# nagadomi/nunif

Hardware: NVIDIA H100
Metric: waifu2x_input_megapixels_per_sec (higher is better)
Workload: dtype f16

## Files before the change

### nunif_b200/csrc/gemm_wgmma.cuh

```cuda
#pragma once
#include "common.cuh"
#include <cuda.h>

namespace nb200 {

enum : int { ACT_NONE = 0, ACT_LRELU01 = 1, ACT_GELU = 2, ACT_RELU = 3 };
enum : int { OUT_NHWC = 0, OUT_PIXSHUF2 = 1, OUT_SPLIT = 2 };

struct GemmParams {
    int B, Ho, Wo, TH, TW, tiles_x, tiles_y;
    int N;
    int taps, cpt;
    int8_t tap_dx[16], tap_dy[16], tap_dyi[16];
    int n_tiles;
    const float* bias;
    int act;
    int out_mode, cout;
    int has_res, res_cy, res_cx;
    int res_before_act;
};

struct GemmMaps {
    CUtensorMap a, b;
    CUtensorMap o[4];
    CUtensorMap r[4];
};

__device__ __forceinline__ uint32_t smem_u32(const void* p) { return (uint32_t)__cvta_generic_to_shared(p); }

__device__ __forceinline__ void mbar_init(uint64_t* bar, uint32_t count) {
    asm volatile("mbarrier.init.shared::cta.b64 [%0], %1;" ::"r"(smem_u32(bar)), "r"(count));
}
__device__ __forceinline__ void mbar_expect_tx(uint64_t* bar, uint32_t bytes) {
    asm volatile("mbarrier.arrive.expect_tx.shared::cta.b64 _, [%0], %1;" ::"r"(smem_u32(bar)), "r"(bytes) : "memory");
}
__device__ __forceinline__ void mbar_arrive(uint64_t* bar) {
    asm volatile("mbarrier.arrive.shared::cta.b64 _, [%0];" ::"r"(smem_u32(bar)) : "memory");
}
static __device__ __noinline__ void mbar_timeout() {
    printf("nb200: mbarrier wait timed out (block %d,%d thread %d)\n", blockIdx.x, blockIdx.y, threadIdx.x);
    __trap();
}
__device__ __forceinline__ void mbar_wait(uint64_t* bar, uint32_t parity) {
    const uint32_t addr = smem_u32(bar);
    uint32_t done = 0;
#pragma unroll 1
    for (uint32_t it = 0; it < (1u << 18); ++it) {
        asm volatile(
            "{\n\t.reg .pred p;\n\t"
            "mbarrier.try_wait.parity.shared::cta.b64 p, [%1], %2, %3;\n\t"
            "selp.u32 %0, 1, 0, p;\n\t}"
            : "=r"(done) : "r"(addr), "r"(parity), "r"(20000u) : "memory");
        if (done) return;
    }
    mbar_timeout();
}
__device__ __forceinline__ void fence_barrier_init() {
    asm volatile("fence.mbarrier_init.release.cluster;" ::: "memory");
    asm volatile("fence.proxy.async.shared::cta;" ::: "memory");
}
__device__ __forceinline__ void tma_load_5d(const CUtensorMap* map, uint64_t* bar, void* dst, int c0, int c1, int c2, int c3, int c4) {
    asm volatile(
        "cp.async.bulk.tensor.5d.shared::cluster.global.tile.mbarrier::complete_tx::bytes [%0], [%1, {%3, %4, %5, %6, %7}], [%2];"
        ::"r"(smem_u32(dst)), "l"(map), "r"(smem_u32(bar)), "r"(c0), "r"(c1), "r"(c2), "r"(c3), "r"(c4) : "memory");
}
__device__ __forceinline__ void tma_load_2d(const CUtensorMap* map, uint64_t* bar, void* dst, int c0, int c1) {
    asm volatile(
        "cp.async.bulk.tensor.2d.shared::cluster.global.tile.mbarrier::complete_tx::bytes [%0], [%1, {%3, %4}], [%2];"
        ::"r"(smem_u32(dst)), "l"(map), "r"(smem_u32(bar)), "r"(c0), "r"(c1) : "memory");
}
__device__ __forceinline__ void tma_load_4d(const CUtensorMap* map, uint64_t* bar, void* dst, int c0, int c1, int c2, int c3) {
    asm volatile(
        "cp.async.bulk.tensor.4d.shared::cluster.global.tile.mbarrier::complete_tx::bytes [%0], [%1, {%3, %4, %5, %6}], [%2];"
        ::"r"(smem_u32(dst)), "l"(map), "r"(smem_u32(bar)), "r"(c0), "r"(c1), "r"(c2), "r"(c3) : "memory");
}
__device__ __forceinline__ void tma_store_4d(const CUtensorMap* map, const void* src, int c0, int c1, int c2, int c3) {
    asm volatile("cp.async.bulk.tensor.4d.global.shared::cta.tile.bulk_group [%0, {%2, %3, %4, %5}], [%1];"
                 ::"l"(map), "r"(smem_u32(src)), "r"(c0), "r"(c1), "r"(c2), "r"(c3) : "memory");
}
__device__ __forceinline__ void tma_store_2d(const CUtensorMap* map, const void* src, int c0, int c1) {
    asm volatile("cp.async.bulk.tensor.2d.global.shared::cta.tile.bulk_group [%0, {%2, %3}], [%1];"
                 ::"l"(map), "r"(smem_u32(src)), "r"(c0), "r"(c1) : "memory");
}
__device__ __forceinline__ void tma_store_commit() { asm volatile("cp.async.bulk.commit_group;" ::: "memory"); }
__device__ __forceinline__ void tma_store_wait_read() { asm volatile("cp.async.bulk.wait_group.read 0;" ::: "memory"); }
__device__ __forceinline__ void fence_async_smem() { asm volatile("fence.proxy.async.shared::cta;" ::: "memory"); }
__device__ __forceinline__ void consumer_bar_sync() { asm volatile("bar.sync 1, 256;" ::: "memory"); }
__device__ __forceinline__ void tma_prefetch_desc(const CUtensorMap* map) {
    asm volatile("prefetch.tensormap [%0];" ::"l"(map) : "memory");
}
__device__ __forceinline__ bool elect_one() {
    uint32_t pred;
    asm volatile(
        "{\n\t.reg .pred p;\n\t"
        "elect.sync _|p, 0xffffffff;\n\t"
        "selp.u32 %0, 1, 0, p;\n\t}"
        : "=r"(pred));
    return pred != 0;
}
__device__ __forceinline__ void wgmma_fence() { asm volatile("wgmma.fence.sync.aligned;" ::: "memory"); }
__device__ __forceinline__ void wgmma_commit() { asm volatile("wgmma.commit_group.sync.aligned;" ::: "memory"); }
template <int N>
__device__ __forceinline__ void wgmma_wait() { asm volatile("wgmma.wait_group.sync.aligned %0;" ::"n"(N) : "memory"); }
template <int K>
__device__ __forceinline__ void wgmma_fence_operands(float (&d)[K]) {
#pragma unroll
    for (int j = 0; j < K; ++j) asm volatile("" : "+f"(d[j])::"memory");
}

template <int SWIZZLE_BYTES>
__device__ __forceinline__ uint64_t make_kmajor_desc(uint32_t saddr) {
    constexpr uint64_t layout = SWIZZLE_BYTES == 128 ? 1 : (SWIZZLE_BYTES == 64 ? 2 : 3);
    constexpr uint64_t sbo = (8 * SWIZZLE_BYTES) >> 4;
    return (uint64_t)((saddr & 0x3FFFF) >> 4) | (1ull << 16) | (sbo << 32) | (layout << 62);
}

template <int N>
__device__ void wgmma_f16(float (&d)[N / 2], uint64_t a, uint64_t b, uint32_t acc);
template <> __device__ __forceinline__ void wgmma_f16<16>(float (&d)[8], uint64_t a, uint64_t b, uint32_t acc) {
    asm volatile("{\n\t.reg .pred p;\n\tsetp.ne.b32 p, %10, 0;\n\t"
                 "wgmma.mma_async.sync.aligned.m64n16k16.f32.f16.f16 {%0, %1, %2, %3, %4, %5, %6, %7}, %8, %9, p, 1, 1, 0, 0;\n\t}"
                 : "+f"(d[0]), "+f"(d[1]), "+f"(d[2]), "+f"(d[3]), "+f"(d[4]), "+f"(d[5]), "+f"(d[6]), "+f"(d[7])
                 : "l"(a), "l"(b), "r"(acc));
}
template <> __device__ __forceinline__ void wgmma_f16<32>(float (&d)[16], uint64_t a, uint64_t b, uint32_t acc) {
    asm volatile("{\n\t.reg .pred p;\n\tsetp.ne.b32 p, %18, 0;\n\t"
                 "wgmma.mma_async.sync.aligned.m64n32k16.f32.f16.f16 {%0, %1, %2, %3, %4, %5, %6, %7, %8, %9, %10, %11, %12, %13, %14, %15}, %16, %17, p, 1, 1, 0, 0;\n\t}"
                 : "+f"(d[0]), "+f"(d[1]), "+f"(d[2]), "+f"(d[3]), "+f"(d[4]), "+f"(d[5]), "+f"(d[6]), "+f"(d[7]), "+f"(d[8]), "+f"(d[9]), "+f"(d[10]), "+f"(d[11]), "+f"(d[12]), "+f"(d[13]), "+f"(d[14]), "+f"(d[15])
                 : "l"(a), "l"(b), "r"(acc));
}
template <> __device__ __forceinline__ void wgmma_f16<48>(float (&d)[24], uint64_t a, uint64_t b, uint32_t acc) {
    asm volatile("{\n\t.reg .pred p;\n\tsetp.ne.b32 p, %26, 0;\n\t"
                 "wgmma.mma_async.sync.aligned.m64n48k16.f32.f16.f16 {%0, %1, %2, %3, %4, %5, %6, %7, %8, %9, %10, %11, %12, %13, %14, %15, %16, %17, %18, %19, %20, %21, %22, %23}, %24, %25, p, 1, 1, 0, 0;\n\t}"
                 : "+f"(d[0]), "+f"(d[1]), "+f"(d[2]), "+f"(d[3]), "+f"(d[4]), "+f"(d[5]), "+f"(d[6]), "+f"(d[7]), "+f"(d[8]), "+f"(d[9]), "+f"(d[10]), "+f"(d[11]), "+f"(d[12]), "+f"(d[13]), "+f"(d[14]), "+f"(d[15]), "+f"(d[16]), "+f"(d[17]), "+f"(d[18]), "+f"(d[19]), "+f"(d[20]), "+f"(d[21]), "+f"(d[22]), "+f"(d[23])
                 : "l"(a), "l"(b), "r"(acc));
}
template <> __device__ __forceinline__ void wgmma_f16<64>(float (&d)[32], uint64_t a, uint64_t b, uint32_t acc) {
    asm volatile("{\n\t.reg .pred p;\n\tsetp.ne.b32 p, %34, 0;\n\t"
// ... 222 lines not shown
```

### nunif_b200/csrc/swin_attention_mma.cu

```cuda
#include "common.cuh"
#include "gemm_wgmma.cuh"
#include "swin_kernels.h"
#include "tmap.h"
#include <map>
#include <mutex>

namespace nb200 {

extern int g_tune[16];

namespace {
constexpr int WS = 6, WTOK = 36, WPAD = 48, HEADS = 6;

__device__ __forceinline__ void mma16816(float (&c)[4], const uint32_t (&a)[4], uint32_t b0, uint32_t b1) {
    asm volatile(
        "mma.sync.aligned.m16n8k16.row.col.f32.f16.f16.f32 {%0,%1,%2,%3}, {%4,%5,%6,%7}, {%8,%9}, {%0,%1,%2,%3};"
        : "+f"(c[0]), "+f"(c[1]), "+f"(c[2]), "+f"(c[3])
        : "r"(a[0]), "r"(a[1]), "r"(a[2]), "r"(a[3]), "r"(b0), "r"(b1));
}
__device__ __forceinline__ void ldmatrix_x2_trans(uint32_t& r0, uint32_t& r1, const void* smem_row) {
    const uint32_t addr = (uint32_t)__cvta_generic_to_shared(smem_row);
    asm volatile("ldmatrix.sync.aligned.m8n8.x2.trans.shared.b16 {%0,%1}, [%2];" : "=r"(r0), "=r"(r1) : "r"(addr));
}
__device__ __forceinline__ uint32_t pack_half2(float a, float b) {
// ... 194 lines not shown
    AttnCtx<D> cx;
    cx.sq = sq; cx.sreg = sreg; cx.bf = bf; cx.hc = hc; cx.g = g; cx.t4 = t4; cx.scale = scale; cx.boundary = boundary;
#pragma unroll
    for (int nt = 0; nt < NKT; ++nt) cx.kbase[nt] = sk + min(nt * 8 + g, WTOK - 1) * LD + hc + 2 * t4;
    cx.vbase[0] = sv + (lane & 15) * LD + hc;
    cx.vbase[1] = sv + (16 + (lane & 15)) * LD + hc;
    cx.vbase[2] = sv + min(32 + (lane & 7), WTOK - 1) * LD + hc;
#pragma unroll 1
    for (int mt = 0; mt < 2; ++mt) attn_mtile<D, LD, false>(cx, mt);
    attn_mtile<D, LD, true>(cx, 2);
    __syncthreads();
    for (int t = rg; t < WTOK; t += RG)
        *reinterpret_cast<uint4*>(out + (size_t)stok[t] * C + vv * 8) = *reinterpret_cast<const uint4*>(sq + t * LD + vv * 8);
}

__global__ void build_bias_frag_kernel(const float* __restrict__ table, float4* __restrict__ frag) {
    const int i = blockIdx.x * blockDim.x + threadIdx.x;
    if (i >= HEADS * 3 * 6 * 32) return;
    const int lane = i & 31, nt = (i >> 5) % 6, mt = (i / (32 * 6)) % 3, head = i / (32 * 6 * 3);
    const int g = lane >> 2, t4 = lane & 3;
    float v[4];
#pragma unroll
    for (int r = 0; r < 4; ++r) {
        const int row = mt * 16 + g + 8 * (r >> 1), col = nt * 8 + 2 * t4 + (r & 1);
        if (col >= WTOK) v[r] = -1e30f;
        else if (row >= WTOK) v[r] = 0.f;
        else {
            const int qy = row / WS, qx = row % WS, ky = col / WS, kx = col % WS;
            v[r] = 1.4426950408889634f * table[((qy - ky + WS - 1) * (2 * WS - 1) + (qx - kx + WS - 1)) * HEADS + head];
        }
    }
    frag[i] = make_float4(v[0], v[1], v[2], v[3]);
}

int build_bias_frag(cudaStream_t st, const float* table, float* frag) {
    build_bias_frag_kernel<<<(HEADS * 3 * 6 * 32 + 255) / 256, 256, 0, st>>>(table, reinterpret_cast<float4*>(frag));
    NB_LAUNCHED();
    return 0;
}

template <int D>
static size_t attn_smem_bytes() {
    constexpr int C = D * HEADS, LD = C + 8;
    return (size_t)3 * WTOK * LD * 2 + (WTOK + WPAD) * 4 + 16;
}

static int set_attn_attrs(const void* func, size_t smem, int carveout) {
    static std::mutex mu;
    static std::map<std::pair<int, const void*>, int> done;
    int dev = 0;
    NB_CUDA(cudaGetDevice(&dev));
    std::lock_guard<std::mutex> lk(mu);
    int& have = done[{dev, func}];
    if (have != carveout) {
        NB_CUDA(cudaFuncSetAttribute(func, cudaFuncAttributeMaxDynamicSharedMemorySize, (int)smem));
        NB_CUDA(cudaFuncSetAttribute(func, cudaFuncAttributePreferredSharedMemoryCarveout, carveout));
        have = carveout;
    }
    return 0;
}

int window_attention(cudaStream_t st, const __half* qkv, const float* bias_frag_f, __half* out, int B, int H, int W, int C,
                     int shift, size_t plane) {
    const float4* bias_table = reinterpret_cast<const float4*>(bias_frag_f);
    NB_CHECK(H % WS == 0 && W % WS == 0, "feature map must be a multiple of the 6x6 window");
    NB_CHECK(C == 96 || C == 192, "window attention supports C=96 (d=16) and C=192 (d=32)");
    if (WS >= H) shift = 0;
    dim3 grid((H / WS) * (W / WS), B);
    ProfScope ps(st, PC_ATTN, (double)B * H * W * C * 4 * 2, (double)B * H * W * C * 3 * 2, (double)B * H * W * C * 2);
    if (C == 96) {
        const int want = g_tune[6] > 0 ? g_tune[6] : 72;
        if (set_attn_attrs((const void*)window_attention_mma_kernel<16>, attn_smem_bytes<16>(), want)) return 1;
        window_attention_mma_kernel<16><<<grid, 192, attn_smem_bytes<16>(), st>>>(qkv, bias_table, out, H, W, shift, plane);
    } else {
        const int want = g_tune[6] > 0 ? g_tune[6] : 86;
        if (set_attn_attrs((const void*)window_attention_mma_kernel<32>, attn_smem_bytes<32>(), want)) return 1;
        window_attention_mma_kernel<32><<<grid, 192, attn_smem_bytes<32>(), st>>>(qkv, bias_table, out, H, W, shift, plane);
    }
    NB_LAUNCHED();
    return 0;
}


constexpr int FA_ROWS = 128, FA_WIN = 3, FA_THREADS = GEMM_CONSUMER_THREADS + 32, FA_SLOT = 96 * 64, FA_STAGES = 4;
constexpr int FA_LD = 32 + 8;
constexpr int FA_CHUNK_BYTES = FA_WIN * 3 * WTOK * FA_LD * 2;

template <int C>
struct FaCfg {
    static constexpr int X_BYTES = FA_ROWS * C * 2;
    static constexpr int SMEM = X_BYTES + FA_STAGES * FA_SLOT + FA_CHUNK_BYTES + FA_WIN * (WTOK + WPAD) * 4 + 2 * FA_STAGES * 8 + 1024;
};

template <int C>
__global__ void __launch_bounds__(FA_THREADS, 2) swin_attn_fused_kernel(const __grid_constant__ CUtensorMap wmap,
                                                                        const __half* __restrict__ x, const float* __restrict__ bqkv,
                                                                        const float4* __restrict__ bias_frag, __half* __restrict__ out,
                                                                        int H, int W, int shift, int nwin) {
    using Cfg = FaCfg<C>;
    constexpr int D = C / HEADS, KB = C / 32, NCH = C / 32, HPC = 32 / D;
    extern __shared__ uint8_t smem_dyn[];
    uint8_t* smem = reinterpret_cast<uint8_t*>((reinterpret_cast<uintptr_t>(smem_dyn) + 1023) & ~(uintptr_t)1023);
    uint8_t* sx = smem;
    uint8_t* ring = smem + Cfg::X_BYTES;
    __half* sqkv = reinterpret_cast<__half*>(ring + FA_STAGES * FA_SLOT);
    int* stok = reinterpret_cast<int*>(reinterpret_cast<uint8_t*>(sqkv) + FA_CHUNK_BYTES);
    int* sreg = stok + FA_WIN * WTOK;
    uint64_t* full = reinterpret_cast<uint64_t*>(sreg + FA_WIN * WPAD);
    uint64_t* empty = full + FA_STAGES;
    const int tid = threadIdx.x, warp = tid >> 5;
    const int nww = W / WS, nwy = H / WS;
    if (tid < FA_WIN * WPAD) {
        const int w = tid / WPAD, t = tid % WPAD, gw = blockIdx.x * FA_WIN + w;
        int reg = -1;
        if (t < WTOK) {
            int tok = -1;
            if (gw < nwin) {
                const int b = gw / (nww * nwy), r = gw % (nww * nwy), wy = r / nww, wx = r % nww;
                const int ry = wy * WS + t / WS, rx = wx * WS + t % WS;
                const int y = (ry + shift) % H, xx = (rx + shift) % W;
                tok = (b * H + y) * W + xx;
                int hr = 0, wr = 0;
                if (shift > 0) {
                    hr = ry < H - WS ? 0 : (ry < H - shift ? 1 : 2);
                    wr = rx < W - WS ? 0 : (rx < W - shift ? 1 : 2);
                }
                reg = hr * 3 + wr;
            }
            stok[w * WTOK + t] = tok;
        }
        sreg[w * WPAD + t] = reg;
    }
    if (tid == GEMM_CONSUMER_THREADS) {
        tma_prefetch_desc(&wmap);
        for (int s = 0; s < FA_STAGES; ++s) {
            mbar_init(&full[s], 1);
            mbar_init(&empty[s], 2);
        }
        fence_barrier_init();
    }
    __syncthreads();
    if (tid == 0) NB_PDL_TRIGGER();

    if (warp == GEMM_CONSUMER_THREADS / 32) {
        if (elect_one()) {
            for (int i = 0; i < NCH * KB; ++i) {
                const int s = i % FA_STAGES, c = i / KB;
                mbar_wait(&empty[s], ((i / FA_STAGES) & 1) ^ 1);
                mbar_expect_tx(&full[s], FA_SLOT);
#pragma unroll
                for (int m = 0; m < 3; ++m)
                    tma_load_2d(&wmap, &full[s], ring + s * FA_SLOT + m * 32 * 64, (i % KB) * 32, m * C + 32 * c);
            }
        }
        return;
    }

    for (int i = tid; i < FA_ROWS * (C / 8); i += GEMM_CONSUMER_THREADS) {
        const int r = i / (C / 8), u = i % (C / 8);
        uint8_t* dst = sx + (u >> 2) * (FA_ROWS * 64) + stage_off<32>(r, u & 3);
        const int tok = r < FA_WIN * WTOK ? stok[r] : -1;
        if (tok >= 0) cp_async16(dst, x + (size_t)tok * C + u * 8);
        else *reinterpret_cast<uint4*>(dst) = make_uint4(0u, 0u, 0u, 0u);
    }
    asm volatile("cp.async.commit_group;" ::: "memory");
    asm volatile("cp.async.wait_group 0;" ::: "memory");
    fence_async_smem();
    consumer_bar_sync();

    const int wg = tid >> 7, t = tid & 127;
    const int row0 = wg * 64 + (t >> 5) * 16 + ((t & 31) >> 2);
    const int cq = 2 * (t & 3);
    const uint32_t a_base = smem_u32(sx) + wg * 64 * 64;
    const int lane = tid & 31, g = lane >> 2, t4 = lane & 3;
    const float scale = ((D == 16) ? 0.25f : 0.17677669529663687f) * 1.4426950408889634f;
#pragma unroll 1
    for (int c = 0; c < NCH; ++c) {
        float acc[48];
#pragma unroll
        for (int j = 0; j < 48; ++j) acc[j] = 0.f;
#pragma unroll 1
        for (int kb = 0; kb < KB; ++kb) {
            const int it = c * KB + kb, s = it % FA_STAGES;
            mbar_wait(&full[s], (it / FA_STAGES) & 1);
            const uint32_t a = a_base + kb * (FA_ROWS * 64), bb = smem_u32(ring + s * FA_SLOT);
            wgmma_fence();
            wgmma_f16<96>(acc, make_kmajor_desc<64>(a), make_kmajor_desc<64>(bb), 1u);
            wgmma_f16<96>(acc, make_kmajor_desc<64>(a + 32), make_kmajor_desc<64>(bb + 32), 1u);
            wgmma_commit();
            wgmma_wait<1>();
            if (kb > 0 && t == 0) mbar_arrive(&empty[(it - 1) % FA_STAGES]);
        }
        wgmma_wait<0>();
        if (t == 0) mbar_arrive(&empty[(c * KB + KB - 1) % FA_STAGES]);
        wgmma_fence_operands(acc);
        consumer_bar_sync();
#pragma unroll
        for (int j = 0; j < 12; ++j) {
            const int m = j >> 2, col = 8 * (j & 3) + cq;
            const float2 bq = __ldg(reinterpret_cast<const float2*>(bqkv + m * C + 32 * c + col));
#pragma unroll
            for (int i = 0; i < 2; ++i) {
                const int r = row0 + 8 * i;
                if (r < FA_WIN * WTOK) {
                    const int w = r / WTOK, tk = r - w * WTOK;
                    *reinterpret_cast<__half2*>(sqkv + ((w * 3 + m) * WTOK + tk) * FA_LD + col) =
                        __floats2half2_rn(acc[4 * j + 2 * i] + bq.x, acc[4 * j + 2 * i + 1] + bq.y);
                }
            }
        }
        consumer_bar_sync();

#pragma unroll 1
        for (int item = warp; item < 3 * FA_WIN * HPC; item += GEMM_CONSUMER_THREADS / 32) {
            const int mt = item / (FA_WIN * HPC), pr = item - mt * (FA_WIN * HPC), w = pr / HPC, hh = pr - w * HPC;
            const int gw = blockIdx.x * FA_WIN + w;
            if (gw >= nwin) continue;
            const int r = gw % (nww * nwy), wy = r / nww, wx = r % nww, head = c * HPC + hh;
            __half* sq = sqkv + w * 3 * WTOK * FA_LD;
            __half* sk = sq + WTOK * FA_LD;
            __half* sv = sk + WTOK * FA_LD;
            AttnCtx<D> cx;
            cx.sq = sq; cx.sreg = sreg + w * WPAD; cx.bf = bias_frag + (size_t)head * (3 * 6 * 32) + lane;
            cx.hc = hh * D; cx.g = g; cx.t4 = t4; cx.scale = scale;
            cx.boundary = shift > 0 && (wy == nwy - 1 || wx == nww - 1);
#pragma unroll
            for (int nt = 0; nt < NKT; ++nt) cx.kbase[nt] = sk + min(nt * 8 + g, WTOK - 1) * FA_LD + cx.hc + 2 * t4;
            cx.vbase[0] = sv + (lane & 15) * FA_LD + cx.hc;
            cx.vbase[1] = sv + (16 + (lane & 15)) * FA_LD + cx.hc;
            cx.vbase[2] = sv + min(32 + (lane & 7), WTOK - 1) * FA_LD + cx.hc;
            if (mt < 2) attn_mtile<D, FA_LD, false>(cx, mt);
            else attn_mtile<D, FA_LD, true>(cx, 2);
            __syncwarp();
            const int nrow = mt < 2 ? 16 : WTOK - 32;
            for (int e = lane; e < nrow * (D / 8); e += 32) {
                const int tk = 16 * mt + e / (D / 8), u = e % (D / 8);
                *reinterpret_cast<uint4*>(out + (size_t)stok[w * WTOK + tk] * C + head * D + u * 8) =
                    *reinterpret_cast<const uint4*>(sq + tk * FA_LD + cx.hc + u * 8);
            }
        }
    }
}

int swin_attn_fused(cudaStream_t st, const __half* x, const __half* wqkv, const float* bqkv, const float* bias_frag_f, __half* att,
                    int B, int H, int W, int C, int shift) {
    NB_CHECK(x && wqkv && bqkv && bias_frag_f && att, "null pointer");
    NB_CHECK(H % WS == 0 && W % WS == 0, "feature map must be a multiple of the 6x6 window");
    NB_CHECK(C == 96 || C == 192, "fused window attention supports C=96 (d=16) and C=192 (d=32)");
    if (WS >= H) shift = 0;
    const long long nwin = (long long)B * (H / WS) * (W / WS);
    NB_CHECK(nwin > 0 && nwin < (1LL << 31), "window count out of range");
    CUtensorMap wmap;
    const cuuint64_t dims[2] = {(cuuint64_t)C, (cuuint64_t)(3 * C)};
    const cuuint64_t strides[1] = {(cuuint64_t)C * 2};
    const cuuint32_t box[2] = {32, 32};
    if (encode(&wmap, wqkv, 2, dims, strides, box, 64)) return 1;
    const double T = (double)B * H * W;
    ProfScope ps(st, PC_FUSED_ATTN, T * 3.0 * C * C * 2 + T * C * 36 * 4, T * C * 2, T * C * 2);
    const unsigned grid = (unsigned)((nwin + FA_WIN - 1) / FA_WIN);
    const float4* bf = reinterpret_cast<const float4*>(bias_frag_f);
    if (C == 96) {
        if (ensure_dyn_smem((const void*)swin_attn_fused_kernel<96>, FaCfg<96>::SMEM)) return 1;
        swin_attn_fused_kernel<96><<<grid, FA_THREADS, FaCfg<96>::SMEM, st>>>(wmap, x, bqkv, bf, att, H, W, shift, (int)nwin);
    } else {
        if (ensure_dyn_smem((const void*)swin_attn_fused_kernel<192>, FaCfg<192>::SMEM)) return 1;
        swin_attn_fused_kernel<192><<<grid, FA_THREADS, FaCfg<192>::SMEM, st>>>(wmap, x, bqkv, bf, att, H, W, shift, (int)nwin);
    }
    NB_LAUNCHED();
    return 0;
}

}
```

### nunif_b200/csrc/swin_block.cu

```cuda
#include "gemm_wgmma.cuh"
#include "swin_kernels.h"
#include "tmap.h"

namespace nb200 {

constexpr int FM_ROWS = 128, FM_STAGES = 5, FM_THREADS = GEMM_CONSUMER_THREADS + 128;
constexpr int FM_PRODUCER_REGS = 40, FM_CONSUMER_REGS = 232;

template <int C>
struct FmCfg {
    static constexpr int KB = C / 32;
    static constexpr int TILE = FM_ROWS * C * 2;
    static constexpr int STAGE = 128 * C;
    static constexpr int SMEM = 2 * TILE + FM_STAGES * STAGE + (2 * FM_STAGES + KB + 1) * 8 + 1024;
};

struct FmMaps {
    CUtensorMap x, att, wp, w1, w2;
};

template <int K>
__device__ __forceinline__ float (&half96(float (&acc)[K], int h))[48] { return *reinterpret_cast<float(*)[48]>(&acc[48 * h]); }

__device__ __forceinline__ void fm_wait(uint64_t* bar, uint32_t parity) {
    const uint32_t addr = smem_u32(bar);
    uint32_t done = 0;
#pragma unroll 1
    for (uint32_t it = 0; it < (1u << 18) && !done; ++it)
        asm volatile(
            "{\n\t.reg .pred p;\n\t"
            "mbarrier.try_wait.parity.shared::cta.b64 p, [%1], %2, %3;\n\t"
            "selp.u32 %0, 1, 0, p;\n\t}"
            : "=r"(done) : "r"(addr), "r"(parity), "r"(20000u) : "memory");
    if (!done) __trap();
}

__device__ __forceinline__ void wgmma_wait_n(int n) {
    if (n == 0) wgmma_wait<0>();
    else wgmma_wait<1>();
}

template <int C, bool PROJ>
__global__ void __launch_bounds__(FM_THREADS, 1) swin_mlp_fused_kernel(const __grid_constant__ FmMaps maps, const float* __restrict__ bp,
                                                                     const float* __restrict__ b1, const float* __restrict__ b2) {
    using Cfg = FmCfg<C>;
    constexpr int KB = Cfg::KB, NP = (KB + 1) / 2, NH = 2 * C / 64, NHALF = C / 96;
    extern __shared__ uint8_t smem_dyn[];
    uint8_t* smem = reinterpret_cast<uint8_t*>((reinterpret_cast<uintptr_t>(smem_dyn) + 1023) & ~(uintptr_t)1023);
    uint8_t* sx = smem;
    uint8_t* satt = smem + Cfg::TILE;
    uint8_t* ring = smem + 2 * Cfg::TILE;
    uint64_t* full = reinterpret_cast<uint64_t*>(ring + FM_STAGES * Cfg::STAGE);
    uint64_t* empty = full + FM_STAGES;
    uint64_t* abar = empty + FM_STAGES;
    uint64_t* xbar = abar + KB;
    const int tid = threadIdx.x, warp = tid >> 5;
    const int row_base = blockIdx.x * FM_ROWS;
    if (tid == GEMM_CONSUMER_THREADS) {
        tma_prefetch_desc(&maps.x);
        tma_prefetch_desc(&maps.w1);
        tma_prefetch_desc(&maps.w2);
        if (PROJ) {
            tma_prefetch_desc(&maps.att);
            tma_prefetch_desc(&maps.wp);
        }
        for (int s = 0; s < FM_STAGES; ++s) {
            mbar_init(&full[s], 1);
            mbar_init(&empty[s], 2);
        }
        for (int kb = 0; kb < KB; ++kb) mbar_init(&abar[kb], 1);
        mbar_init(xbar, 1);
        fence_barrier_init();
    }
    __syncthreads();

    if (warp >= GEMM_CONSUMER_THREADS / 32) {
        asm volatile("setmaxnreg.dec.sync.aligned.u32 %0;" ::"n"(FM_PRODUCER_REGS));
        if (warp == GEMM_CONSUMER_THREADS / 32 && elect_one()) {
            bool acts = false;
            auto load_acts = [&]() {
                asm volatile("griddepcontrol.wait;" ::: "memory");
                if (PROJ)
                    for (int kb = 0; kb < KB; ++kb) {
                        mbar_expect_tx(&abar[kb], FM_ROWS * 64);
                        tma_load_2d(&maps.att, &abar[kb], satt + kb * (FM_ROWS * 64), kb * 32, row_base);
                    }
                mbar_expect_tx(xbar, Cfg::TILE);
                for (int kb = 0; kb < KB; ++kb) tma_load_2d(&maps.x, xbar, sx + kb * (FM_ROWS * 64), kb * 32, row_base);
                acts = true;
            };
            int it = 0;
            auto push = [&](const CUtensorMap* m, int k0, int n0, int rows, int nbox) {
                if (it == FM_STAGES) load_acts();
                const int s = it % FM_STAGES;
                fm_wait(&empty[s], ((it / FM_STAGES) & 1) ^ 1);
                mbar_expect_tx(&full[s], nbox * rows * 64);
                for (int b = 0; b < nbox; ++b) tma_load_2d(m, &full[s], ring + s * Cfg::STAGE + b * rows * 64, k0 + 32 * b, n0);
                ++it;
            };
            if (PROJ)
                for (int j = 0; j < NP; ++j) push(&maps.wp, 64 * j, 0, C, min(2, KB - 2 * j));
            push(&maps.w1, 0, 0, 64, KB);
            for (int hc = 0; hc < NH; ++hc) {
                if (hc + 1 < NH) push(&maps.w1, 0, (hc + 1) * 64, 64, KB);
                push(&maps.w2, hc * 64, 0, C, 2);
            }
            if (!acts) load_acts();
        }
        return;
    }

    asm volatile("setmaxnreg.inc.sync.aligned.u32 %0;" ::"n"(FM_CONSUMER_REGS));
    const int wg = tid >> 7, t = tid & 127;
    const int row0 = wg * 64 + (t >> 5) * 16 + ((t & 31) >> 2);
    const int cq = 2 * (t & 3);
    const uint32_t x_base = smem_u32(sx) + wg * 64 * 64, att_base = smem_u32(satt) + wg * 64 * 64;
    int it = 0, pending = 0;
    auto take = [&]() -> uint32_t {
        const int s = it % FM_STAGES;
        fm_wait(&full[s], (it / FM_STAGES) & 1);
        return smem_u32(ring + s * Cfg::STAGE);
    };
    auto commit = [&]() {
        wgmma_commit();
        ++it;
        ++pending;
    };
    auto retire = [&](int n) {
        wgmma_wait_n(n);
#pragma unroll
        for (int k = 0; k < FM_STAGES; ++k)
            if (k < pending - n && t == 0) mbar_arrive(&empty[(it - pending + k) % FM_STAGES]);
        pending = min(pending, n);
    };

    if (PROJ) {
        float acc[C / 2];
#pragma unroll
        for (int j = 0; j < C / 2; ++j) acc[j] = 0.f;
        wgmma_fence_operands(acc);
#pragma unroll
        for (int j = 0; j < NP; ++j) {
            const uint32_t bb = take();
#pragma unroll
            for (int kb = 2 * j; kb < 2 * j + 2 && kb < KB; ++kb) fm_wait(&abar[kb], 0);
            wgmma_fence();
#pragma unroll
            for (int kb = 2 * j; kb < 2 * j + 2 && kb < KB; ++kb) {
                const uint32_t a = att_base + kb * (FM_ROWS * 64), b = bb + (kb - 2 * j) * (C * 64);
#pragma unroll
                for (int s = 0; s < 2; ++s)
#pragma unroll
                    for (int h = 0; h < NHALF; ++h)
                        wgmma_f16<96>(half96(acc, h), make_kmajor_desc<64>(a + 32 * s), make_kmajor_desc<64>(b + h * 96 * 64 + 32 * s), 1u);
            }
            commit();
            retire(1);
        }
        retire(0);
        wgmma_fence_operands(acc);
        fm_wait(xbar, 0);
#pragma unroll
        for (int j = 0; j < C / 8; ++j) {
            const int col = 8 * j + cq;
            const float2 bq = __ldg(reinterpret_cast<const float2*>(bp + col));
#pragma unroll
            for (int i = 0; i < 2; ++i) {
                __half2* p = reinterpret_cast<__half2*>(sx + sw64_off<FM_ROWS>(row0 + 8 * i, col));
                const float2 xv = __half22float2(*p);
                *p = __floats2half2_rn(xv.x + (acc[4 * j + 2 * i] + bq.x), xv.y + (acc[4 * j + 2 * i + 1] + bq.y));
            }
        }
        fence_async_smem();
        asm volatile("bar.sync %0, 128;" ::"r"(2 + wg) : "memory");
    } else {
        fm_wait(xbar, 0);
    }

    float oacc[C / 2];
#pragma unroll
    for (int j = 0; j < C / 2; ++j) oacc[j] = 0.f;
    wgmma_fence_operands(oacc);
    float hacc[2][32];
    uint32_t af[4][4];
    auto fc1 = [&](float (&h)[32]) {
#pragma unroll
        for (int j = 0; j < 32; ++j) h[j] = 0.f;
        wgmma_fence_operands(h);
        const uint32_t bb = take();
        wgmma_fence();
#pragma unroll
        for (int kb = 0; kb < KB; ++kb) {
            const uint32_t a = x_base + kb * (FM_ROWS * 64), b = bb + kb * (64 * 64);
            wgmma_f16<64>(h, make_kmajor_desc<64>(a), make_kmajor_desc<64>(b), 1u);
            wgmma_f16<64>(h, make_kmajor_desc<64>(a + 32), make_kmajor_desc<64>(b + 32), 1u);
        }
        commit();
    };
    fc1(hacc[0]);
#pragma unroll
    for (int hc = 0; hc < NH; ++hc) {
        const int buf = hc & 1;
        if (hc + 1 < NH) fc1(hacc[buf ^ 1]);
        retire(hc + 1 < NH ? 1 : 0);
        wgmma_fence_operands(hacc[buf]);
#pragma unroll
        for (int kk = 0; kk < 4; ++kk)
#pragma unroll
            for (int q = 0; q < 4; ++q) {
                const int j = 2 * kk + (q >> 1), i = q & 1;
                const float2 bq = __ldg(reinterpret_cast<const float2*>(b1 + 64 * hc + 8 * j + cq));
                const __half2 h = __floats2half2_rn(gelu_erf(hacc[buf][4 * j + 2 * i] + bq.x), gelu_erf(hacc[buf][4 * j + 2 * i + 1] + bq.y));
                af[kk][q] = *reinterpret_cast<const uint32_t*>(&h);
            }
        const uint32_t bb = take();
        wgmma_fence();
#pragma unroll
        for (int kb = 0; kb < 2; ++kb)
#pragma unroll
            for (int s = 0; s < 2; ++s)
#pragma unroll
                for (int h = 0; h < NHALF; ++h)
                    wgmma_f16_rs96(half96(oacc, h), af[2 * kb + s], make_kmajor_desc<64>(bb + kb * (C * 64) + h * 96 * 64 + 32 * s), 1u);
        commit();
    }
    retire(0);
    wgmma_fence_operands(oacc);
#pragma unroll
    for (int j = 0; j < C / 8; ++j) {
        const int col = 8 * j + cq;
        const float2 bq = __ldg(reinterpret_cast<const float2*>(b2 + col));
#pragma unroll
        for (int i = 0; i < 2; ++i) {
            __half2* p = reinterpret_cast<__half2*>(sx + sw64_off<FM_ROWS>(row0 + 8 * i, col));
            const float2 xv = __half22float2(*p);
            *p = __floats2half2_rn(xv.x + (oacc[4 * j + 2 * i] + bq.x), xv.y + (oacc[4 * j + 2 * i + 1] + bq.y));
        }
    }
    fence_async_smem();
    consumer_bar_sync();
    if (tid == 0) {
        for (int kb = 0; kb < KB; ++kb) tma_store_2d(&maps.x, sx + kb * (FM_ROWS * 64), kb * 32, row_base);
        tma_store_commit();
        tma_store_wait_read();
    }
}

static int map2d(CUtensorMap* m, const void* base, int cols, long long rows, int box_rows) {
    const cuuint64_t dims[2] = {(cuuint64_t)cols, (cuuint64_t)rows};
    const cuuint64_t strides[1] = {(cuuint64_t)cols * 2};
    const cuuint32_t box[2] = {32, (cuuint32_t)box_rows};
    return encode(m, base, 2, dims, strides, box, 64);
}

template <int C, bool PROJ>
static int launch_mlp(cudaStream_t st, unsigned grid, const FmMaps& maps, const float* bp, const float* b1, const float* b2) {
    if (ensure_dyn_smem((const void*)swin_mlp_fused_kernel<C, PROJ>, FmCfg<C>::SMEM)) return 1;
    cudaLaunchConfig_t cfg = {};
    cfg.gridDim = dim3(grid); cfg.blockDim = dim3(FM_THREADS); cfg.dynamicSmemBytes = FmCfg<C>::SMEM;
// ... 49 lines not shown
```

### profiles/ab_swin_attn.py

```python
#!/usr/bin/env python
import argparse
import ctypes
import json
import os
import statistics
import subprocess
import sys
import tempfile

ROOT = os.path.dirname(os.path.dirname(os.path.abspath(__file__)))
sys.path.insert(0, ROOT)

SHAPES = [(240, 96), (120, 192), (60, 192), (240, 192)]
BATCH = 16
REPS = 7
WINDOW_MS = 60.0
FA_THREADS = 288
KERNEL = "_ZN5nb20022swin_attn_fused_kernelILi{C}EEEv14CUtensorMap_stPK6__halfPKfPK6float4PS2_iiii"


def load(path):
    from nunif_b200 import _lib
    lib = ctypes.CDLL(os.path.abspath(path))
    for name in ("nb200_last_error", "nb200_check_device", "nb200_swin_attn_fused_f16"):
        res, args = _lib.SIGNATURES[name]
        getattr(lib, name).restype, getattr(lib, name).argtypes = res, args
    return lib


def check(lib, rc):
    if rc != 0:
        raise RuntimeError(lib.nb200_last_error().decode("utf-8", "replace"))


def call(lib, t, shift):
    import torch
    x, wqkv, bqkv, table, att = t
    B, H, W, C = x.shape
    p = lambda v: ctypes.c_void_p(v.data_ptr())
    check(lib, lib.nb200_swin_attn_fused_f16(p(x), p(wqkv), p(bqkv), p(table), p(att), B, H, W, C, shift,
                                             ctypes.c_void_p(torch.cuda.current_stream().cuda_stream)))


def inputs(H, C, shift, dev):
    import torch
    g = torch.Generator(device="cpu").manual_seed(H * 1000 + C + shift)
    x = torch.randn(BATCH, H, H, C, generator=g).half().to(dev)
    wqkv = (torch.randn(3 * C, C, generator=g) / C ** 0.5).half().to(dev)
    bqkv = (0.1 * torch.randn(3 * C, generator=g)).to(dev)
    table = (0.5 * torch.randn(121, 6, generator=g)).to(dev)
    return x, wqkv, bqkv, table


def window_ms(lib, t, shift, n):
    import torch
    e0, e1 = torch.cuda.Event(enable_timing=True), torch.cuda.Event(enable_timing=True)
    e0.record()
    for _ in range(n):
        call(lib, t, shift)
    e1.record()
    e1.synchronize()
    return e0.elapsed_time(e1) / n


def launch_smem(libs, dev):
    import torch
    from torch.profiler import ProfilerActivity, profile
    out = {}
    with tempfile.TemporaryDirectory() as d:
        for tag, lib in libs.items():
            for C in (96, 192):
                x, wqkv, bqkv, table = inputs(12, C, 0, dev)
                t = (x, wqkv, bqkv, table, torch.empty_like(x))
                with profile(activities=[ProfilerActivity.CUDA]) as prof:
                    call(lib, t, 0)
                    torch.cuda.synchronize()
                path = os.path.join(d, f"{tag}{C}.json")
                prof.export_chrome_trace(path)
                ev = [e for e in json.load(open(path))["traceEvents"]
                      if e.get("cat") == "kernel" and "swin_attn_fused_kernel" in e.get("name", "")]
                a = ev[0]["args"]
                out[(tag, C)] = {"smem": int(a["shared memory"]), "regs_trace": int(a["registers per thread"])}
    return out


def occupancy(so_path, C, smem):
    name = KERNEL.format(C=C)
    cuobjdump = os.path.join(os.environ.get("CUDA_HOME", "/usr/local/cuda"), "bin", "cuobjdump")
    with tempfile.TemporaryDirectory() as d:
        subprocess.run([cuobjdump, "-xelf", "all", os.path.abspath(so_path)], cwd=d, check=True, capture_output=True)
        image = next(b for b in (open(os.path.join(d, f), "rb").read() for f in sorted(os.listdir(d))) if name.encode() in b)
    cu = ctypes.CDLL("libcuda.so.1")

    def ck(rc):
        if rc != 0:
            raise RuntimeError(f"CUDA driver error {rc}")
    mod, fn = ctypes.c_void_p(), ctypes.c_void_p()
    ck(cu.cuModuleLoadData(ctypes.byref(mod), ctypes.c_char_p(image)))
    try:
        ck(cu.cuModuleGetFunction(ctypes.byref(fn), mod, name.encode()))
        ck(cu.cuFuncSetAttribute(fn, 8, ctypes.c_int(smem)))
        regs, n = ctypes.c_int(), ctypes.c_int()
        ck(cu.cuFuncGetAttribute(ctypes.byref(regs), 4, fn))
        ck(cu.cuOccupancyMaxActiveBlocksPerMultiprocessor(ctypes.byref(n), fn, FA_THREADS, ctypes.c_size_t(smem)))
    finally:
        cu.cuModuleUnload(mod)
    return regs.value, n.value


def device_info(index):
    q = subprocess.run(["nvidia-smi", "-i", str(index), "--query-gpu=name,power.limit,clocks.max.sm", "--format=csv,noheader"],
                       capture_output=True, text=True)
    return q.stdout.strip()


def main():
    ap = argparse.ArgumentParser(description=__doc__, formatter_class=argparse.RawDescriptionHelpFormatter)
    ap.add_argument("--base", required=True, help="the build to compare against (libnunif_b200.so)")
    ap.add_argument("--new", default=os.path.join(ROOT, "nunif_b200", "libnunif_b200.so"), help="default: this tree's build")
    ap.add_argument("--out", default=None, help="also write the JSON result here")
    args = ap.parse_args()
    import torch
    from bench import ClockSampler
    dev = torch.device("cuda:0")
    torch.cuda.init()
    torch.zeros(1, device=dev)
    paths = {"base": args.base, "new": args.new}
    libs = {k: load(v) for k, v in paths.items()}
    for lib in libs.values():
        check(lib, lib.nb200_check_device(0))
    info = {"device": torch.cuda.get_device_name(dev), "nvidia_smi": device_info(0), "paths": paths}
    print(f"# {info['device']} | name, power limit, max SM clock: {info['nvidia_smi']}")

    kern = []
    try:
        for (tag, C), s in sorted(launch_smem(libs, dev).items()):
            regs, ctas = occupancy(paths[tag], C, s["smem"])
            kern.append({"build": tag, "C": C, "regs": regs, "dyn_smem": s["smem"], "ctas_per_sm": ctas})
            print(f"# {tag:4s} swin_attn_fused_kernel<{C}>: {regs} registers, {s['smem']} B shared memory/CTA, {ctas} CTA(s)/SM")
    except Exception as e:
        kern.append({"error": f"{type(e).__name__}: {e}"})
        print(f"# occupancy query failed: {type(e).__name__}: {e}")

    rows = []
    with torch.inference_mode(), ClockSampler(0) as clocks:
        for H, C in SHAPES:
            for shift in (0, 3):
                x, wqkv, bqkv, table = inputs(H, C, shift, dev)
                t = {k: (x, wqkv, bqkv, table, torch.full_like(x, 7.0)) for k in libs}
                for k, lib in libs.items():
                    for _ in range(3):
                        call(lib, t[k], shift)
                torch.cuda.synchronize()
                equal = torch.equal(t["base"][4], t["new"][4])
                diff = float((t["base"][4].float() - t["new"][4].float()).abs().max())
                est = max(window_ms(libs["base"], t["base"], shift, 2), window_ms(libs["new"], t["new"], shift, 2))
                n = max(3, int(WINDOW_MS / max(est, 1e-3)))
                ms = {k: [] for k in libs}
                for r in range(REPS):
                    for k in (("base", "new") if r % 2 == 0 else ("new", "base")):
                        ms[k].append(window_ms(libs[k], t[k], shift, n))
                row = {"B": BATCH, "H": H, "W": H, "C": C, "shift": shift, "calls_per_window": n, "equal": equal, "max_abs_diff": diff}
                for k in libs:
                    row[k] = {"median_ms": statistics.median(ms[k]), "min_ms": min(ms[k]), "max_ms": max(ms[k])}
                row["new_over_base"] = row["new"]["median_ms"] / row["base"]["median_ms"]
                rows.append(row)
                b, nw = row["base"], row["new"]
                print(f"{BATCH}x{H}x{H}x{C} shift {shift}: base {b['median_ms']:.4f} ms [{b['min_ms']:.4f}, {b['max_ms']:.4f}]  "
                      f"new {nw['median_ms']:.4f} ms [{nw['min_ms']:.4f}, {nw['max_ms']:.4f}]  new/base {row['new_over_base']:.3f}  "
                      f"outputs {'identical' if equal else f'DIFFER (max |d| {diff:g})'}", flush=True)
                del t, x
    result = {"info": info, "clocks": clocks.summary(), "kernels": kern, "shapes": rows,
              "all_equal": all(r["equal"] for r in rows)}
    print(json.dumps(result))
    if args.out:
        os.makedirs(os.path.dirname(os.path.abspath(args.out)), exist_ok=True)
        with open(args.out, "w") as fh:
            json.dump(result, fh, indent=1)
    return 0 if result["all_equal"] else 1


if __name__ == "__main__":
    sys.exit(main())
```

Before: 54.01.

## Deepen fused attention TMA ring, add PDL launch, unroll k-loop, interleave warp items

Raises the weight ring in the fused Swin attention kernel from 4 to 6 stages and fully unrolls the k-block loop. Launches the kernel with programmatic stream serialization and places griddepcontrol.wait before the consumers read activations, so the prologue can overlap the previous kernel. Assigns attention work items to warps in a serpentine order to balance load, and moves the trapping mbarrier wait into the shared header. The extra stages increase shared memory per CTA, which could lower the number of CTAs resident per SM.

```diff
diff --git a/nunif_b200/csrc/gemm_wgmma.cuh b/nunif_b200/csrc/gemm_wgmma.cuh
--- a/nunif_b200/csrc/gemm_wgmma.cuh
+++ b/nunif_b200/csrc/gemm_wgmma.cuh
@@ -54,6 +54,18 @@
         if (done) return;
     }
     mbar_timeout();
+}
+__device__ __forceinline__ void mbar_wait_trap(uint64_t* bar, uint32_t parity) {
+    const uint32_t addr = smem_u32(bar);
+    uint32_t done = 0;
+#pragma unroll 1
+    for (uint32_t it = 0; it < (1u << 18) && !done; ++it)
+        asm volatile(
+            "{\n\t.reg .pred p;\n\t"
+            "mbarrier.try_wait.parity.shared::cta.b64 p, [%1], %2, %3;\n\t"
+            "selp.u32 %0, 1, 0, p;\n\t}"
+            : "=r"(done) : "r"(addr), "r"(parity), "r"(20000u) : "memory");
+    if (!done) __trap();
 }
 __device__ __forceinline__ void fence_barrier_init() {
     asm volatile("fence.mbarrier_init.release.cluster;" ::: "memory");
diff --git a/nunif_b200/csrc/swin_attention_mma.cu b/nunif_b200/csrc/swin_attention_mma.cu
--- a/nunif_b200/csrc/swin_attention_mma.cu
+++ b/nunif_b200/csrc/swin_attention_mma.cu
@@ -300,7 +300,8 @@
 }
 
 
-constexpr int FA_ROWS = 128, FA_WIN = 3, FA_THREADS = GEMM_CONSUMER_THREADS + 32, FA_SLOT = 96 * 64, FA_STAGES = 4;
+constexpr int FA_ROWS = 128, FA_WIN = 3, FA_THREADS = GEMM_CONSUMER_THREADS + 32, FA_SLOT = 96 * 64;
+constexpr int FA_STAGES = 6;
 constexpr int FA_LD = 32 + 8;
 constexpr int FA_CHUNK_BYTES = FA_WIN * 3 * WTOK * FA_LD * 2;
 
@@ -364,7 +365,7 @@
         if (elect_one()) {
             for (int i = 0; i < NCH * KB; ++i) {
                 const int s = i % FA_STAGES, c = i / KB;
-                mbar_wait(&empty[s], ((i / FA_STAGES) & 1) ^ 1);
+                mbar_wait_trap(&empty[s], ((i / FA_STAGES) & 1) ^ 1);
                 mbar_expect_tx(&full[s], FA_SLOT);
 #pragma unroll
                 for (int m = 0; m < 3; ++m)
@@ -373,6 +374,8 @@
         }
         return;
     }
+
+    asm volatile("griddepcontrol.wait;" ::: "memory");
 
     for (int i = tid; i < FA_ROWS * (C / 8); i += GEMM_CONSUMER_THREADS) {
         const int r = i / (C / 8), u = i % (C / 8);
@@ -397,10 +400,10 @@
         float acc[48];
 #pragma unroll
         for (int j = 0; j < 48; ++j) acc[j] = 0.f;
-#pragma unroll 1
+#pragma unroll
         for (int kb = 0; kb < KB; ++kb) {
             const int it = c * KB + kb, s = it % FA_STAGES;
-            mbar_wait(&full[s], (it / FA_STAGES) & 1);
+            mbar_wait_trap(&full[s], (it / FA_STAGES) & 1);
             const uint32_t a = a_base + kb * (FA_ROWS * 64), bb = smem_u32(ring + s * FA_SLOT);
             wgmma_fence();
             wgmma_f16<96>(acc, make_kmajor_desc<64>(a), make_kmajor_desc<64>(bb), 1u);
@@ -430,7 +433,7 @@
         consumer_bar_sync();
 
 #pragma unroll 1
-        for (int item = warp; item < 3 * FA_WIN * HPC; item += GEMM_CONSUMER_THREADS / 32) {
+        for (int rd = 0, item = warp; item < 3 * FA_WIN * HPC; ++rd, item = 8 * rd + ((rd & 1) ? 7 - warp : warp)) {
             const int mt = item / (FA_WIN * HPC), pr = item - mt * (FA_WIN * HPC), w = pr / HPC, hh = pr - w * HPC;
             const int gw = blockIdx.x * FA_WIN + w;
             if (gw >= nwin) continue;
@@ -458,6 +461,22 @@
             }
         }
     }
+}
+
+template <int C>
+static int launch_attn(cudaStream_t st, unsigned grid, const CUtensorMap& wmap, const __half* x, const float* bqkv, const float4* bf,
+                       __half* att, int H, int W, int shift, int nwin) {
+    if (ensure_dyn_smem((const void*)swin_attn_fused_kernel<C>, FaCfg<C>::SMEM)) return 1;
+    cudaLaunchConfig_t cfg = {};
+    cfg.gridDim = dim3(grid); cfg.blockDim = dim3(FA_THREADS); cfg.dynamicSmemBytes = FaCfg<C>::SMEM;
+    cfg.stream = st;
+    cudaLaunchAttribute at[1];
+    at[0].id = cudaLaunchAttributeProgrammaticStreamSerialization;
+    at[0].val.programmaticStreamSerializationAllowed = 1;
+    cfg.attrs = at; cfg.numAttrs = 1;
+    NB_CUDA(cudaLaunchKernelEx(&cfg, swin_attn_fused_kernel<C>, wmap, x, bqkv, bf, att, H, W, shift, nwin));
+    NB_LAUNCHED();
+    return 0;
 }
 
 int swin_attn_fused(cudaStream_t st, const __half* x, const __half* wqkv, const float* bqkv, const float* bias_frag_f, __half* att,
@@ -477,15 +496,8 @@
     ProfScope ps(st, PC_FUSED_ATTN, T * 3.0 * C * C * 2 + T * C * 36 * 4, T * C * 2, T * C * 2);
     const unsigned grid = (unsigned)((nwin + FA_WIN - 1) / FA_WIN);
     const float4* bf = reinterpret_cast<const float4*>(bias_frag_f);
-    if (C == 96) {
-        if (ensure_dyn_smem((const void*)swin_attn_fused_kernel<96>, FaCfg<96>::SMEM)) return 1;
-        swin_attn_fused_kernel<96><<<grid, FA_THREADS, FaCfg<96>::SMEM, st>>>(wmap, x, bqkv, bf, att, H, W, shift, (int)nwin);
-    } else {
-        if (ensure_dyn_smem((const void*)swin_attn_fused_kernel<192>, FaCfg<192>::SMEM)) return 1;
-        swin_attn_fused_kernel<192><<<grid, FA_THREADS, FaCfg<192>::SMEM, st>>>(wmap, x, bqkv, bf, att, H, W, shift, (int)nwin);
-    }
-    NB_LAUNCHED();
-    return 0;
-}
-
-}
+    if (C == 96) return launch_attn<96>(st, grid, wmap, x, bqkv, bf, att, H, W, shift, (int)nwin);
+    return launch_attn<192>(st, grid, wmap, x, bqkv, bf, att, H, W, shift, (int)nwin);
+}
+
+}
diff --git a/nunif_b200/csrc/swin_block.cu b/nunif_b200/csrc/swin_block.cu
--- a/nunif_b200/csrc/swin_block.cu
+++ b/nunif_b200/csrc/swin_block.cu
@@ -21,19 +21,6 @@
 
 template <int K>
 __device__ __forceinline__ float (&half96(float (&acc)[K], int h))[48] { return *reinterpret_cast<float(*)[48]>(&acc[48 * h]); }
-
-__device__ __forceinline__ void fm_wait(uint64_t* bar, uint32_t parity) {
-    const uint32_t addr = smem_u32(bar);
-    uint32_t done = 0;
-#pragma unroll 1
-    for (uint32_t it = 0; it < (1u << 18) && !done; ++it)
-        asm volatile(
-            "{\n\t.reg .pred p;\n\t"
-            "mbarrier.try_wait.parity.shared::cta.b64 p, [%1], %2, %3;\n\t"
-            "selp.u32 %0, 1, 0, p;\n\t}"
-            : "=r"(done) : "r"(addr), "r"(parity), "r"(20000u) : "memory");
-    if (!done) __trap();
-}
 
 __device__ __forceinline__ void wgmma_wait_n(int n) {
     if (n == 0) wgmma_wait<0>();
@@ -93,7 +80,7 @@
             auto push = [&](const CUtensorMap* m, int k0, int n0, int rows, int nbox) {
                 if (it == FM_STAGES) load_acts();
                 const int s = it % FM_STAGES;
-                fm_wait(&empty[s], ((it / FM_STAGES) & 1) ^ 1);
+                mbar_wait_trap(&empty[s], ((it / FM_STAGES) & 1) ^ 1);
                 mbar_expect_tx(&full[s], nbox * rows * 64);
                 for (int b = 0; b < nbox; ++b) tma_load_2d(m, &full[s], ring + s * Cfg::STAGE + b * rows * 64, k0 + 32 * b, n0);
                 ++it;
@@ -118,7 +105,7 @@
     int it = 0, pending = 0;
     auto take = [&]() -> uint32_t {
         const int s = it % FM_STAGES;
-        fm_wait(&full[s], (it / FM_STAGES) & 1);
+        mbar_wait_trap(&full[s], (it / FM_STAGES) & 1);
         return smem_u32(ring + s * Cfg::STAGE);
     };
     auto commit = [&]() {
@@ -143,7 +130,7 @@
         for (int j = 0; j < NP; ++j) {
             const uint32_t bb = take();
 #pragma unroll
-            for (int kb = 2 * j; kb < 2 * j + 2 && kb < KB; ++kb) fm_wait(&abar[kb], 0);
+            for (int kb = 2 * j; kb < 2 * j + 2 && kb < KB; ++kb) mbar_wait_trap(&abar[kb], 0);
             wgmma_fence();
 #pragma unroll
             for (int kb = 2 * j; kb < 2 * j + 2 && kb < KB; ++kb) {
@@ -159,7 +146,7 @@
         }
         retire(0);
         wgmma_fence_operands(acc);
-        fm_wait(xbar, 0);
+        mbar_wait_trap(xbar, 0);
 #pragma unroll
         for (int j = 0; j < C / 8; ++j) {
             const int col = 8 * j + cq;
@@ -174,7 +161,7 @@
         fence_async_smem();
         asm volatile("bar.sync %0, 128;" ::"r"(2 + wg) : "memory");
     } else {
-        fm_wait(xbar, 0);
+        mbar_wait_trap(xbar, 0);
     }
 
     float oacc[C / 2];
diff --git a/profiles/ab_swin_attn.py b/profiles/ab_swin_attn.py
--- a/profiles/ab_swin_attn.py
+++ b/profiles/ab_swin_attn.py
@@ -15,7 +15,6 @@
 BATCH = 16
 REPS = 7
 WINDOW_MS = 60.0
-FA_THREADS = 288
 KERNEL = "_ZN5nb20022swin_attn_fused_kernelILi{C}EEEv14CUtensorMap_stPK6__halfPKfPK6float4PS2_iiii"
 
 
@@ -80,11 +79,12 @@
                 ev = [e for e in json.load(open(path))["traceEvents"]
                       if e.get("cat") == "kernel" and "swin_attn_fused_kernel" in e.get("name", "")]
                 a = ev[0]["args"]
-                out[(tag, C)] = {"smem": int(a["shared memory"]), "regs_trace": int(a["registers per thread"])}
+                out[(tag, C)] = {"smem": int(a["shared memory"]), "regs_trace": int(a["registers per thread"]),
+                                 "threads": int(a["block"][0] * a["block"][1] * a["block"][2])}
     return out
 
 
-def occupancy(so_path, C, smem):
+def occupancy(so_path, C, smem, threads):
     name = KERNEL.format(C=C)
     cuobjdump = os.path.join(os.environ.get("CUDA_HOME", "/usr/local/cuda"), "bin", "cuobjdump")
     with tempfile.TemporaryDirectory() as d:
@@ -102,7 +102,7 @@
         ck(cu.cuFuncSetAttribute(fn, 8, ctypes.c_int(smem)))
         regs, n = ctypes.c_int(), ctypes.c_int()
         ck(cu.cuFuncGetAttribute(ctypes.byref(regs), 4, fn))
-        ck(cu.cuOccupancyMaxActiveBlocksPerMultiprocessor(ctypes.byref(n), fn, FA_THREADS, ctypes.c_size_t(smem)))
+        ck(cu.cuOccupancyMaxActiveBlocksPerMultiprocessor(ctypes.byref(n), fn, threads, ctypes.c_size_t(smem)))
     finally:
         cu.cuModuleUnload(mod)
     return regs.value, n.value
@@ -135,9 +135,9 @@
     kern = []
     try:
         for (tag, C), s in sorted(launch_smem(libs, dev).items()):
-            regs, ctas = occupancy(paths[tag], C, s["smem"])
-            kern.append({"build": tag, "C": C, "regs": regs, "dyn_smem": s["smem"], "ctas_per_sm": ctas})
-            print(f"# {tag:4s} swin_attn_fused_kernel<{C}>: {regs} registers, {s['smem']} B shared memory/CTA, {ctas} CTA(s)/SM")
+            regs, ctas = occupancy(paths[tag], C, s["smem"], s["threads"])
+            kern.append({"build": tag, "C": C, "regs": regs, "threads": s["threads"], "dyn_smem": s["smem"], "ctas_per_sm": ctas})
+            print(f"# {tag:4s} swin_attn_fused_kernel<{C}>: {s['threads']} threads, {regs} registers, {s['smem']} B shared memory/CTA, {ctas} CTA(s)/SM")
     except Exception as e:
         kern.append({"error": f"{type(e).__name__}: {e}"})
         print(f"# occupancy query failed: {type(e).__name__}: {e}")
```

New measurement: 55.31 (median of 6 runs). +2.4%, better.
